# JuliaStats/Klara.jl

Measured on AMD Instinct MI355X. Metric: MCMC transitions/sec (whole node), 100-dim Gaussian, 65k chains, higher is better.
Workload: dtype f64

## Files before the change

### klara.jl_amd/csrc/detmath.h

```cpp
#ifndef KLARA_DETMATH_H
#define KLARA_DETMATH_H

#ifndef __HIPCC_RTC__
#include <stdint.h>
#endif

#if defined(__HIPCC__)
#define KD_FN __host__ __device__ __forceinline__
#else
#define KD_FN static inline __attribute__((always_inline))
#endif

KD_FN uint64_t kd_d2u(double x) { uint64_t u; __builtin_memcpy(&u, &x, 8); return u; }
KD_FN double   kd_u2d(uint64_t u) { double x; __builtin_memcpy(&x, &u, 8); return x; }
KD_FN double   kd_fma(double a, double b, double c) { return __builtin_fma(a, b, c); }

#define KD_PHILOX_M0 0xD2511F53u
#define KD_PHILOX_M1 0xCD9E8D57u
#define KD_PHILOX_W0 0x9E3779B9u
#define KD_PHILOX_W1 0xBB67AE85u

typedef struct { uint32_t x, y, z, w; } kd_u32x4;

#if defined(__HIP_DEVICE_COMPILE__)
// ... 374 lines not shown
    double d = kd_fma(-g, g, y);
    g = kd_fma(d, h, g);
    d = kd_fma(-g, g, y);
    return kd_fma(d, h, g);
#else
    return __builtin_sqrt(y);
#endif
}

KD_FN uint64_t kd_angle_bits20(uint32_t wb)
{
#if defined(__HIP_DEVICE_COMPILE__)
    return ((uint64_t)__builtin_amdgcn_alignbit(0x3ffu, wb, 12) << 32) | 0x80000000ull;
#else
    return ((uint64_t)(0x3ff00000u | (wb >> 12)) << 32) | 0x80000000ull;
#endif
}
#define KD_SCREM_ENTRIES 4096
#define KD_SCREM_BYTES (KD_SCREM_ENTRIES * 16)
KD_FN void kd_sincos_rem_entry(uint32_t m, double* sy_out, double* dc_out)
{
    kd_sincos_rem(kd_angle_bits20(m << 12), sy_out, dc_out);
}
#if defined(__HIPCC__)
typedef double kd_screm_t __attribute__((ext_vector_type(2)));
extern __shared__ __attribute__((aligned(16))) kd_screm_t kd_screm_lds[];
__device__ __forceinline__ void kd_sincos_rem_to_lds()
{
    for (int m = (int)threadIdx.x; m < KD_SCREM_ENTRIES; m += (int)blockDim.x) {
        double sy, dc;
        kd_sincos_rem_entry((uint32_t)m, &sy, &dc);
        kd_screm_lds[m] = kd_screm_t{ sy, dc };
    }
}
__device__ __forceinline__ void kd_sincos2pi_tab20(uint32_t wb, double* sn, double* cs)
{
    const uint32_t k = wb >> 12;
    const kd_screm_t r = kd_screm_lds[k & (KD_SCREM_ENTRIES - 1u)];
    kd_sincos_rotate(k >> 12, r.x, r.y, sn, cs);
}
#endif
#if defined(__HIPCC__)
template <bool TAB>
KD_FN void kd_normal_pair_w_t(uint32_t wa, uint32_t wb, double* z0, double* z1, double* u1_out, double* logu1_out)
#else
KD_FN void kd_normal_pair_w(uint32_t wa, uint32_t wb, double* z0, double* z1, double* u1_out, double* logu1_out)
#endif
{
    const double u1 = kd_u44(wa, wb);
    const double lg = kd_log_u01(u1);
    const double rad = kd_sqrt_radicand(-2.0 * lg);
    double sn, cs;
#if defined(__HIPCC__)
    if constexpr (TAB) kd_sincos2pi_tab20(wb, &sn, &cs);
    else
#endif
    kd_sincos2pi_bits(kd_angle_bits20(wb), &sn, &cs);
    *z0 = rad * cs;
    *z1 = rad * sn;
    *u1_out = u1;
    *logu1_out = lg;
}
#if defined(__HIPCC__)
KD_FN void kd_normal_pair_w(uint32_t wa, uint32_t wb, double* z0, double* z1, double* u1_out, double* logu1_out)
{
    kd_normal_pair_w_t<false>(wa, wb, z0, z1, u1_out, logu1_out);
}
#endif
#if defined(__HIPCC__)
typedef struct {
    kd_screm_t lg, rot, rem;
    double z; int k; double u1;
} kd_pair_reads;
__device__ __forceinline__ void kd_normal_pair_issue(uint32_t wa, uint32_t wb, kd_pair_reads* r)
{
    uint32_t i;
    r->u1 = kd_u44(wa, wb);
    kd_log_u01_reduce(r->u1, &i, &r->k, &r->z);
    const uint32_t k = wb >> 12;
    r->lg = *(const kd_screm_t*)&KD_LOGTAB(2 * i);
    r->rot = *(const kd_screm_t*)&KD_SCTAB(2 * (k >> 12));
    r->rem = kd_screm_lds[k & (KD_SCREM_ENTRIES - 1u)];
}
__device__ __forceinline__ void kd_normal_pair_finish(const kd_pair_reads* r, double* z0, double* z1, double* u1_out, double* logu1_out)
{
    const double lg = kd_log_u01_finish(r->z, r->k, r->lg.x, r->lg.y);
    const double rad = kd_sqrt_radicand(-2.0 * lg);
    double sn, cs;
    kd_sincos_rotate_entry(r->rot.x, r->rot.y, r->rem.x, r->rem.y, &sn, &cs);
    *z0 = rad * cs;
    *z1 = rad * sn;
    *u1_out = r->u1;
    *logu1_out = lg;
}
#endif

KD_FN uint32_t kd_pair_block(uint32_t p) { return (p & 7u) | ((p >> 4) << 3); }
KD_FN uint32_t kd_pair_half(uint32_t p) { return (p >> 3) & 1u; }
KD_FN void kd_normal_pair_at(uint64_t seed, uint64_t chain, uint64_t transition, uint32_t p, uint32_t nreal,
                             double* z0, double* z1, double* u1_out, double* logu1_out)
{
    const int real = p < nreal;
    const int half = real && kd_pair_half(p) != 0u;
    const kd_u32x4 b = kd_stream_block(seed, chain, transition, real ? kd_pair_block(p) : p);
    kd_normal_pair_w(half ? b.z : b.x, half ? b.w : b.y, z0, z1, u1_out, logu1_out);
}
KD_FN double kd_accept_uniform(kd_u32x4 b) { return kd_u44(b.x, b.y); }

KD_FN double kd_uniform_xy(kd_u32x4 b) { return kd_u52(b.x, b.y); }
KD_FN double kd_uniform_zw(kd_u32x4 b) { return kd_u52(b.z, b.w); }
KD_FN uint32_t kd_slice_attempt_slot(uint32_t base, uint32_t a) { return base | ((a + 1u) >> 1); }
KD_FN double kd_slice_attempt_uniform(uint64_t seed, uint64_t chain, uint64_t transition, uint32_t base, uint32_t a)
{
    const kd_u32x4 b = kd_stream_block(seed, chain, transition, kd_slice_attempt_slot(base, a));
    return (a & 1u) ? kd_uniform_xy(b) : kd_uniform_zw(b);
}

#endif
```

### klara.jl_amd/csrc/klara_diagt.h

```cpp
#pragma once
#include "klara_kernels.h"

#ifndef KLARA_DIAGT_Q
#define KLARA_DIAGT_Q 8
#endif
#define KLARA_DIAGT_CPW (64 / KLARA_DIAGT_Q)
#ifndef KLARA_DT_FENCE_EVERY
#define KLARA_DT_FENCE_EVERY 2
#endif
#ifndef KLARA_DT_SLICE_WF
#define KLARA_DT_SLICE_WF 4
#endif
#ifndef KLARA_DT_W1
#define KLARA_DT_W1 4
#endif
#ifndef KLARA_Q4_MALA_WF
#define KLARA_Q4_MALA_WF 3
#endif
#ifndef KLARA_Q4_SCTAB_WF
#define KLARA_Q4_SCTAB_WF 3
#endif
#ifndef KLARA_DT_WF
#define KLARA_DT_WF 2
#endif
#ifdef KLARA_DT_PERSISTENT
#define KLARA_DT_GROUP_LOOP for (long long grp = kl.group0 + wave0; grp < kl.group_end && grp * CPW < p.nchains; grp += nwaves)
#else
#define KLARA_DT_GROUP_LOOP const long long grp = kl.group0 + wave0; if (grp < kl.group_end && grp * CPW < p.nchains)
#endif
#define KLARA_DT_PAIR_FENCE(pi) do { if (KLARA_DT_FENCE_EVERY > 0 && ((pi) + 1) % KLARA_DT_FENCE_EVERY == 0) __builtin_amdgcn_sched_barrier(0); } while (0)

struct KAuto {
    const int* cell_in;
    int* cell_out;
    unsigned long long* acc_ctr;
    int* mirror;
    unsigned long long thr_work;
    int my_mode;
    int fanout;
    int launch_idx;
};
#define KLARA_AUTO_NONE KAuto{ nullptr, nullptr, nullptr, nullptr, 0ull, 0, 1, 0 }

__device__ __forceinline__ unsigned wave_sum_u32(unsigned v)
{
#pragma unroll
    for (int m = 1; m < 64; m <<= 1) v += (unsigned)__builtin_amdgcn_ds_bpermute((int)((((unsigned)threadIdx.x & 63u) ^ (unsigned)m) << 2), (int)v);
    return v;
}
__shared__ unsigned klara_auto_wg[2];
__device__ __forceinline__ void auto_begin()
{
    if (threadIdx.x < 2) klara_auto_wg[threadIdx.x] = 0u;
}
__device__ __forceinline__ void auto_finish(const KAuto& ka, unsigned wave_acc)
{
    if (ka.acc_ctr == nullptr) return;
    const unsigned tot = wave_sum_u32(wave_acc);
    if ((threadIdx.x & 63) == 0) {
        atomicAdd(&klara_auto_wg[0], tot);
        if (atomicAdd(&klara_auto_wg[1], 1u) != (blockDim.x >> 6) - 1) return;
        const unsigned long long wg_tot = atomicAdd(&klara_auto_wg[0], 0u);
        const unsigned long long old = atomicAdd(ka.acc_ctr, (1ull << 40) | wg_tot);
        if ((old >> 40) == (unsigned long long)gridDim.x - 1) {
            const unsigned long long total = (old & ((1ull << 40) - 1)) + wg_tot;
            *ka.acc_ctr = 0ull;
            const int mode = (total << 16) > ka.thr_work ? 1 : 0;
            if (ka.cell_out != nullptr) for (int k = 0; k < ka.fanout; ++k) ka.cell_out[2 * k] = mode;
            if (ka.mirror != nullptr) {
                for (int k = 0; k < ka.fanout; ++k) {
                    __hip_atomic_store(ka.mirror + 4 * k + 1, (int)(total > 0x7fffffffull ? 0x7fffffffull : total), __ATOMIC_RELAXED, __HIP_MEMORY_SCOPE_SYSTEM);
                    __hip_atomic_store(ka.mirror + 4 * k, mode, __ATOMIC_RELAXED, __HIP_MEMORY_SCOPE_SYSTEM);
                    __hip_atomic_store(ka.mirror + 4 * k + 2, ka.launch_idx, __ATOMIC_RELEASE, __HIP_MEMORY_SCOPE_SYSTEM);
                }
            }
        }
    }
}

template <int NP, int Q>
struct PairCtx {
    int lane, q, cw;
    unsigned off0;
    bool last_ok;
// ... 148 lines not shown
        }
#pragma unroll
        for (int k = 0; k < CH; ++k) {
            if (p0 + k < NP) {
                const int p = p0 + k;
                const unsigned o = fold ? pair_off<NP, Q>(c, p) : KLARA_BUF_OOB;
                const double s0 = __builtin_bit_cast(double, kd_uint2{ ts[k].x, ts[k].y }) + hf * x[2 * p];
                const double s1 = __builtin_bit_cast(double, kd_uint2{ ts[k].z, ts[k].w }) + hf * x[2 * p + 1];
                const double q0 = __builtin_bit_cast(double, kd_uint2{ tq[k].x, tq[k].y }) + hf * (x[2 * p] * x[2 * p]);
                const double q1 = __builtin_bit_cast(double, kd_uint2{ tq[k].z, tq[k].w }) + hf * (x[2 * p + 1] * x[2 * p + 1]);
                const kd_uint2 a = __builtin_bit_cast(kd_uint2, s0), b = __builtin_bit_cast(kd_uint2, s1);
                const kd_uint2 e = __builtin_bit_cast(kd_uint2, q0), f = __builtin_bit_cast(kd_uint2, q1);
                if (p < NP - 1) {
                    __builtin_amdgcn_raw_buffer_store_b128(kd_uint4{ a.x, a.y, b.x, b.y }, wsum, o, 0, 0);
                    __builtin_amdgcn_raw_buffer_store_b128(kd_uint4{ e.x, e.y, f.x, f.y }, wsq, o, 0, 0);
                } else {
                    const unsigned o1 = (fold && c.last_full) ? o + 8u : KLARA_BUF_OOB;
                    __builtin_amdgcn_raw_buffer_store_b64(a, wsum, o, 0, 0); __builtin_amdgcn_raw_buffer_store_b64(b, wsum, o1, 0, 0);
                    __builtin_amdgcn_raw_buffer_store_b64(e, wsq, o, 0, 0); __builtin_amdgcn_raw_buffer_store_b64(f, wsq, o1, 0, 0);
                }
            }
        }
    }
    held = fold ? 0 : held;
}

template <int NP, int Q>
__device__ __forceinline__ void load_pair_param(const PairCtx<NP, Q>& c, const gdouble* base, int D, double dflt, double (&v)[2 * NP])
{
#pragma unroll
    for (int p = 0; p < NP; ++p) {
        const int i = 2 * (p * Q + c.q);
        v[2 * p] = dflt; v[2 * p + 1] = dflt;
        if (base != nullptr && i < D) v[2 * p] = base[i];
        if (base != nullptr && i + 1 < D) v[2 * p + 1] = base[i + 1];
    }
}

template <int Q> struct PairShare {
    static constexpr int STEP = Q <= 8 ? 8 / Q : 0;
    static constexpr bool second(int p) { return STEP != 0 && ((p / (STEP ? STEP : 1)) & 1) != 0; }
};
template <int NP, int Q>
__device__ __forceinline__ void pair_words(const PairCtx<NP, Q>& c, unsigned long long seed, unsigned long long gchain,
                                           unsigned long long t, int p, uint32_t (&stash)[4], uint32_t& wa, uint32_t& wb)
{
    constexpr int STEP = PairShare<Q>::STEP, S1 = STEP ? STEP : 1;
    if (PairShare<Q>::second(p)) {
        wa = stash[2 * (p % S1)]; wb = stash[2 * (p % S1) + 1];
    } else {
        const uint32_t idx = (uint32_t)(p * Q + c.q);
        const bool pad = p == NP - 1 && !c.last_ok;
        const kd_u32x4 b = kd_stream_block(seed, gchain, t, pad ? idx : kd_pair_block(idx));
        if constexpr (STEP != 0) {
            wa = b.x; wb = b.y;
            stash[2 * (p % S1)] = b.z; stash[2 * (p % S1) + 1] = b.w;
        } else {
            const bool hb = !pad && kd_pair_half(idx) != 0u;
            wa = hb ? b.z : b.x; wb = hb ? b.w : b.y;
        }
    }
}
template <int NP, int Q, bool SCTAB = false>
__device__ __forceinline__ void pair_normals(const PairCtx<NP, Q>& c, unsigned long long seed, unsigned long long gchain,
                                             unsigned long long t, int p, uint32_t (&stash)[4], double& z0, double& z1, double& u1, double& lg1)
{
    uint32_t wa, wb;
    pair_words<NP, Q>(c, seed, gchain, t, p, stash, wa, wb);
    kd_normal_pair_w_t<SCTAB>(wa, wb, &z0, &z1, &u1, &lg1);
    KLARA_PIN(z0); KLARA_PIN(z1);
    if (p == NP - 1 && !c.last_ok) z0 = 0.0;
    if (p == NP - 1 && !c.last_full) z1 = 0.0;
}
template <int NP, int Q>
__device__ __forceinline__ void pair_issue(const PairCtx<NP, Q>& c, unsigned long long seed, unsigned long long gchain,
                                           unsigned long long t, int p, uint32_t (&stash)[4], kd_pair_reads& rd)
{
    uint32_t wa, wb;
    pair_words<NP, Q>(c, seed, gchain, t, p, stash, wa, wb);
    kd_normal_pair_issue(wa, wb, &rd);
    __builtin_amdgcn_sched_barrier(0);
}
template <int NP, int Q>
__device__ __forceinline__ void pair_finish(const PairCtx<NP, Q>& c, int p, const kd_pair_reads& rd, double& z0, double& z1, double& u1, double& lg1)
{
    kd_normal_pair_finish(&rd, &z0, &z1, &u1, &lg1);
    KLARA_PIN(z0); KLARA_PIN(z1);
    if (p == NP - 1 && !c.last_ok) z0 = 0.0;
    if (p == NP - 1 && !c.last_full) z1 = 0.0;
}

template <int V> struct kd_int { static constexpr int value = V; };
template <int FROM, int TO, class F>
__device__ __forceinline__ void kd_static_for(F&& f)
{
    if constexpr (FROM < TO) { f(kd_int<FROM>{}); kd_static_for<FROM + 1, TO>(f); }
}

template <bool UNITW>
__device__ __forceinline__ void diag_elem(double x, double w, double m2w, double m, double& term, double& grad)
{
    const double dd = UNITW ? x : x - m;
    term = UNITW ? dd * dd : w * (dd * dd);
    grad = UNITW ? -2.0 * dd : m2w * dd;
}

template <int SAMPLER, int NP, int Q, bool ONESTEP, bool TUNE, bool SCTAB = false>
__host__ __device__ constexpr int diagt_min_waves()
{
    return SCTAB && Q == 4 && NP > 8 ? KLARA_Q4_SCTAB_WF
         : NP <= 8 ? (ONESTEP && SAMPLER != KLARA_SAMPLER_HMC ? KLARA_DT_W1 : KLARA_DT_WF)
                   : (Q == 4 && NP <= 13 && !TUNE ? (SAMPLER == KLARA_SAMPLER_MALA ? KLARA_Q4_MALA_WF : 2) : 1);
}

#ifndef KLARA_SCTAB_MIN_STEPS
#define KLARA_SCTAB_MIN_STEPS 8
#endif
template <int SAMPLER, int NP, int Q, bool ONESTEP, bool UNITW, bool MON, bool TUNE>
__host__ __device__ constexpr bool diagt_sctab()
{
    return SAMPLER == KLARA_SAMPLER_MALA && ((Q == 4 && NP == 13) || (Q == 8 && NP == 7)) && !ONESTEP && UNITW && MON && !TUNE;
}
#ifndef KLARA_Q4_SCTAB_WG
#define KLARA_Q4_SCTAB_WG 256
#endif
template <int Q, bool SCTAB>
__host__ __device__ constexpr int diagt_wg_threads() { return SCTAB && Q == 4 ? KLARA_Q4_SCTAB_WG : 256; }
#ifndef KLARA_Q4_KEPT_MEANS
#define KLARA_Q4_KEPT_MEANS 0
#endif
#ifndef KLARA_Q8_KEPT_MEANS
#define KLARA_Q8_KEPT_MEANS 0
#endif
template <int SAMPLER, int NP, int Q, bool UNITW, bool TUNE, bool SCTAB>
__host__ __device__ constexpr int diagt_kept_means()
{
    return SCTAB && SAMPLER == KLARA_SAMPLER_MALA && UNITW && !TUNE ? (Q == 4 ? KLARA_Q4_KEPT_MEANS : Q == 8 ? KLARA_Q8_KEPT_MEANS : 0) : 0;
}

#ifdef KLARA_USER_PAIR_TARGET
#define KLARA_PAIR_CALL(a, b, P, g0, g1) klara_user_pair((a), (b), (P), D, (const double*)p.cdata, (long long)p.cndata, (g0), (g1))
#else
#define KLARA_PAIR_CALL(a, b, P, g0, g1) 0.0
#endif
template <int SAMPLER, int NP, int Q, bool ONESTEP, bool UNITW, bool MON, bool TUNE = false, bool DA = false, bool USERPAIR = false, bool SCTAB = false>
__global__ __launch_bounds__((diagt_wg_threads<Q, SCTAB>()), (SAMPLER == KLARA_SAMPLER_SLICE && NP <= 8 && !MON && !TUNE ? KLARA_DT_SLICE_WF : diagt_min_waves<SAMPLER, NP, Q, ONESTEP, TUNE, SCTAB>()))
void k_diagt(const KParams* __restrict__ pp, const KLaunch kl, const KAuto ka)
{
#ifndef KLARA_USER_PAIR_TARGET
    static_assert(!USERPAIR, "pair closures exist in run-time compiled translation units only");
#endif
    static_assert(!USERPAIR || (UNITW && Q >= 8), "pair closures: 8 or more lanes per chain");
    static_assert(!SCTAB || (!ONESTEP && !USERPAIR && SAMPLER != KLARA_SAMPLER_SLICE), "the remainder table: fused launches of the built-in MH / MALA / HMC kernels");
    if (ka.cell_in != nullptr && *ka.cell_in != ka.my_mode) return;
    static_assert(!(ONESTEP && (MON || TUNE)), "monitored / tuned jobs run the committing kernel");
    static_assert(!DA || (TUNE && SAMPLER == KLARA_SAMPLER_HMC), "dual averaging: tuned HMC");
    constexpr bool PLAIN = !TUNE;
    constexpr int E = 2 * NP, CPW = 64 / Q;
    constexpr bool NEEDG = SAMPLER == KLARA_SAMPLER_MALA || SAMPLER == KLARA_SAMPLER_HMC;
    constexpr bool SLICE = SAMPLER == KLARA_SAMPLER_SLICE;
    constexpr int KM = diagt_kept_means<SAMPLER, NP, Q, UNITW, TUNE, SCTAB>();
    static_assert(KM >= 0 && KM <= E, "kept drift means: a prefix of the lane's elements");
    static_assert(!(SLICE && ONESTEP), "the slice sampler moves every chain: it runs the committing kernel");
    constexpr bool MEMSUM = MON && !TUNE && Q == 4 && (SAMPLER == KLARA_SAMPLER_MH || SAMPLER == KLARA_SAMPLER_MALA);
    const KParams& p = *pp;
    __shared__ __attribute__((aligned(16))) double lds_w[UNITW ? 2 : 2 * NP * Q];
    __shared__ __attribute__((aligned(16))) double lds_mu[UNITW ? 2 : 2 * NP * Q];
    __shared__ __attribute__((aligned(16))) double lds_m2w[UNITW ? 2 : 2 * NP * Q];
    if (!UNITW) {
        for (int i = (int)threadIdx.x; i < 2 * NP * Q; i += (int)blockDim.x) {
            lds_w[i] = (p.gw != nullptr && i < p.D) ? p.gw[i] : 1.0;
            lds_mu[i] = (p.gmu != nullptr && i < p.D) ? p.gmu[i] : 0.0;
            lds_m2w[i] = -2.0 * lds_w[i];
        }
    }
    auto_begin();
    if constexpr (SCTAB) kd_sincos_rem_to_lds();
    kd_tables_to_lds();
    if (p.clock_probe != nullptr && blockIdx.x == (gridDim.x >> 1) && threadIdx.x == 0) {
        p.clock_probe[2] = __builtin_amdgcn_s_memtime(); p.clock_probe[3] = __builtin_amdgcn_s_memrealtime();
    }
    const int D = p.D;
    const PairCtx<NP, Q> cx = make_pctx<NP, Q>(D);
    const int nsteps = ONESTEP ? 1 : kl.nsteps;
    guchar* const accept_out = p.accept != nullptr ? p.accept + kl.t0 * (unsigned long long)p.nchains : nullptr;

    double sig[E];
    const auto wv = [&](int e) { return UNITW ? 1.0 : lds_w[2 * ((e >> 1) * Q + cx.q) + (e & 1)]; };
    const auto mv = [&](int e) { return UNITW ? 0.0 : lds_mu[2 * ((e >> 1) * Q + cx.q) + (e & 1)]; };
    const auto m2wv = [&](int e) { return UNITW ? -2.0 : lds_m2w[2 * ((e >> 1) * Q + cx.q) + (e & 1)]; };
    const auto wvl = [&](int e) { return UNITW ? 1.0 : *(volatile const double*)&lds_w[2 * ((e >> 1) * Q + cx.q) + (e & 1)]; };
    const auto mvl = [&](int e) { return UNITW ? 0.0 : *(volatile const double*)&lds_mu[2 * ((e >> 1) * Q + cx.q) + (e & 1)]; };
    const auto m2wvl = [&](int e) { return UNITW ? -2.0 : *(volatile const double*)&lds_m2w[2 * ((e >> 1) * Q + cx.q) + (e & 1)]; };
    if (SAMPLER == KLARA_SAMPLER_MH) load_pair_param<NP, Q>(cx, p.vecparam, D, 1.0, sig);
    const double gconst = USERPAIR ? 0.0 : p.gconst;

    const int acc_slot = (D + 1) >> 1;
    const bool acc_free = acc_slot < NP * Q && !PairShare<Q>::second(NP - 1);
    const int acc_lane = (cx.lane - cx.q) + (acc_slot & (Q - 1));

    const long long nwaves = (long long)gridDim.x * (blockDim.x >> 6);
    const long long wave0 = __builtin_amdgcn_readfirstlane((int)(blockIdx.x * (blockDim.x >> 6) + (threadIdx.x >> 6)));
    unsigned wave_acc = 0;
    KLARA_DT_GROUP_LOOP {
        const long long first_chain = grp * CPW;
        const long long left = p.nchains - first_chain;
        const int here = left < CPW ? (int)left : CPW;
        const bool chain_ok = cx.cw < here;
        const long long chain = first_chain + cx.cw;
        const unsigned long long gchain = (unsigned long long)(p.chain_offset + chain);
        const __amdgpu_buffer_rsrc_t wx = group_window(p.X, first_chain, here, D);
        const __amdgpu_buffer_rsrc_t wg = group_window(p.GR, first_chain, here, D);

        double x[E];
        load_pairs<NP, Q>(cx, wx, x);
        const auto late_ctx = [&]() -> PairCtx<NP, Q> {
            if constexpr (SCTAB && Q == 4) {
                int l = (int)__builtin_amdgcn_mbcnt_hi(~0u, __builtin_amdgcn_mbcnt_lo(~0u, 0u));
                KLARA_PIN(l);
                return make_pctx_at<NP, Q>(D, l & 63);
            } else return cx;
        };
        const auto user_pair = [&](int pi, double a, double b, double& nt, double& g0, double& g1) {
            double u0 = 0.0, u1 = 0.0, u = 0.0;
            const bool ok0 = pi < NP - 1 || cx.last_ok, ok1 = pi < NP - 1 || cx.last_full;
            if (ok0) u = KLARA_PAIR_CALL(a, b, pi * Q + cx.q, &u0, &u1);
            nt = ok0 ? -u : 0.0; g0 = ok0 ? u0 : 0.0; g1 = ok1 ? u1 : 0.0;
        };
        const auto grad_of = [&](const double (&v)[E], double (&out)[E]) {
            if constexpr (USERPAIR) {
#pragma unroll
                for (int pi = 0; pi < NP; ++pi) { double nt; user_pair(pi, v[2 * pi], v[2 * pi + 1], nt, out[2 * pi], out[2 * pi + 1]); }
            } else {
#pragma unroll
                for (int e = 0; e < E; ++e) { double term_; diag_elem<UNITW>(v[e], wv(e), m2wv(e), mv(e), term_, out[e]); }
            }
        };
        double lt = p.LT[chain_ok ? chain : 0];
        unsigned long long nacc = 0;
        bool stuck = false;
        const bool do_sum = MON && p.sum != nullptr;
        double sm[MEMSUM ? 2 : E], sq[MEMSUM ? 2 : E];
        bool sums_loaded = false;
        long long held = 0;
        __amdgpu_buffer_rsrc_t wsum = wx, wsq = wx;
        if (do_sum) {
#pragma unroll
            for (int e = 0; e < (MEMSUM ? 2 : E); ++e) { sm[e] = 0.0; sq[e] = 0.0; }
            wsum = group_window(p.sum, first_chain, here, D); wsq = group_window(p.sumsq, first_chain, here, D);
            held = p.held[chain_ok ? chain : 0];
        }
        int sphase = kl.save_phase0;
        long long scol = kl.save_col0;
        const bool per_chain_tune = KCNT && !KPOOLED;
        const long long c0 = chain_ok ? chain : 0;
        TuneRegs tn;
        if (per_chain_tune) tn = { p.tune_step[c0], p.tune_accepted[c0], p.tune_proposed[c0], p.tune_totproposed[c0], 0, 0.0, 0.0 };
        else if (KPOOLED) tn = { p.tune_step[0], p.tune_accepted[0], 0, 0, 0, 0.0, 0.0 };
        else tn = { DA ? p.tune_step[c0] : p.step0, 0, 0, 0, 0, 0.0, 0.0 };
        if (DA) { tn.epsbar = p.da_epsbar[c0]; tn.hbar = p.da_hbar[c0]; }
        const long long acc0 = tn.accepted;
        tn.phase = per_chain_tune ? (int)(tn.proposed % p.period) : 0;

        struct { unsigned long long seed; long long hist_cols, held_inc; int thinning, acc_free, save_lo, save_hi; double sqrt_step0, half_inv_step0; } lc = {};
        if constexpr (SCTAB) {
            lc.seed = p.seed; lc.hist_cols = p.hist_cols; lc.thinning = (int)p.thinning;
            lc.held_inc = __builtin_amdgcn_readfirstlane(do_sum ? 1 : 0); lc.sqrt_step0 = p.sqrt_step0;
            KLARA_PIN_S(lc.seed); KLARA_PIN_S(lc.hist_cols); KLARA_PIN_S(lc.thinning);
            KLARA_PIN_S(lc.held_inc); KLARA_PIN_S(lc.sqrt_step0);
            const kd_uint2 hih = __builtin_bit_cast(kd_uint2, 0.5 * p.inv_step0);
            lc.half_inv_step0 = __builtin_bit_cast(double, kd_uint2{ (uint32_t)__builtin_amdgcn_readfirstlane((int)hih.x), (uint32_t)__builtin_amdgcn_readfirstlane((int)hih.y) });
            KLARA_PIN_S(lc.half_inv_step0);
            lc.acc_free = __builtin_amdgcn_readfirstlane(acc_free ? 1 : 0);
            KLARA_PIN_S(lc.acc_free);
            const long long lo = (long long)p.burnin - (long long)kl.t0, hi = (long long)p.nsteps_total - (long long)kl.t0;
            lc.save_lo = (int)(lo < 0 ? 0 : lo > nsteps ? nsteps : lo); lc.save_hi = (int)(hi < 0 ? 0 : hi > nsteps ? nsteps : hi);
            KLARA_PIN_S(lc.save_lo); KLARA_PIN_S(lc.save_hi);
        }
#define KLARA_LC(f) (SCTAB ? lc.f : p.f)
        double dm[KM > 0 ? KM : 1];
        const double neg_h_kept = KM > 0 ? -tn.step : 0.0;
        if constexpr (KM > 0) {
#pragma unroll
            for (int e = 0; e < KM; ++e) dm[e] = x[e] + neg_h_kept * x[e];
        }
        for (int s = 0; s < nsteps; ++s) {
            const unsigned long long t = kl.t0 + (unsigned long long)s;
            if (KCNT) tune_count_proposal(p, tn);
            double xp[E];
            const auto put_xp = [&](int pi, double a, double b) { xp[2 * pi] = a; xp[2 * pi + 1] = b; };
            constexpr int NR = Q == 4 ? 2 : 1;
            double red[3 * NR] = {}, red1[1], red2[2];
            double u_last = 0.5, lg_last = 0.0;
            uint32_t nstash[4] = { 0u, 0u, 0u, 0u };
            bool acc;
            double ltp, a_da = 0.0;

            constexpr bool ZFIRST = (ONESTEP || Q != 4) && SAMPLER != KLARA_SAMPLER_HMC && !SLICE;
            double z[ZFIRST ? E : 2];
            kd_pair_reads rd[2];
            if (ZFIRST) {
                if constexpr (SCTAB) pair_issue<NP, Q>(cx, KLARA_LC(seed), gchain, t, 0, nstash, rd[0]);
#pragma unroll
                for (int pi = 0; pi < NP; ++pi) {
                    if constexpr (SCTAB) {
                        if (pi + 1 < NP) pair_issue<NP, Q>(cx, KLARA_LC(seed), gchain, t, pi + 1, nstash, rd[(pi + 1) & 1]);
                        pair_finish<NP, Q>(cx, pi, rd[pi & 1], z[2 * pi], z[2 * pi + 1], u_last, lg_last);
                        __builtin_amdgcn_sched_barrier(0);
                    } else {
                        pair_normals<NP, Q, SCTAB>(cx, KLARA_LC(seed), gchain, t, pi, nstash, z[2 * pi], z[2 * pi + 1], u_last, lg_last);
                        KLARA_DT_PAIR_FENCE(pi);
                    }
                }
            }
            if constexpr (SLICE) {
                if (do_sum && __any(held > 0))
                    diagt_fold<NP, Q>(cx, wsum, wsq, held > 0, sums_loaded, held, x, sm, sq);
            }
            if (SLICE) {
                acc = true;
                const __amdgpu_buffer_rsrc_t wwid = __builtin_amdgcn_make_buffer_rsrc((void*)p.vecparam, 0, D * 8, 0x00020000);
#pragma unroll
                for (int e = 0; e < E; ++e) {
                    const int i = 2 * ((e >> 1) * Q + cx.q) + (e & 1);
                    const bool live = chain_ok && i < D;
                    const uint32_t base = (uint32_t)(live ? i : 0) << KLARA_SLICE_ATT_BITS;
                    const kd_u32x4 b0 = kd_stream_block(KLARA_LC(seed), gchain, t, base);
                    const double lgu = kd_log_u01(kd_uniform_xy(b0));
                    const double ru = kd_uniform_zw(b0);
                    const double wi_t = UNITW ? 1.0 : wv(e), mi_t = UNITW ? 0.0 : mv(e);
                    const double xi = x[e], wd = __builtin_bit_cast(double, __builtin_amdgcn_raw_buffer_load_b64(wwid, (unsigned)(live ? i : 0) * 8u, 0, 0));
                    double tcur, gd_;
                    if constexpr (USERPAIR) { double g1_; user_pair(e >> 1, x[e & ~1], x[e | 1], tcur, gd_, g1_); }
                    else diag_elem<UNITW>(xi, wi_t, -2.0 * wi_t, mi_t, tcur, gd_);
                    double Li = xi - ru * wd;
                    double Ri = xi + (1.0 - ru) * wd;
                    const auto term_of = [&](double cand) -> double {
                        double tc, gd;
                        if constexpr (USERPAIR) { double g1; user_pair(e >> 1, (e & 1) ? x[e & ~1] : cand, (e & 1) ? cand : x[e | 1], tc, gd, g1); }
                        else diag_elem<UNITW>(cand, wi_t, -2.0 * wi_t, mi_t, tc, gd);
                        return tc;
                    };
                    if (p.stepout) {
                        double dl = tcur - term_of(Li);
                        int guard = 0;
                        while (true) {
                            bool go = live && !stuck && (dl > lgu);
                            if (go && ++guard > KLARA_SLICE_MAX_ATT) { stuck = true; go = false; }
                            if (!__any(go)) break;
                            const double Ln = Li - wd;
                            const double dn = tcur - term_of(go ? Ln : Li);
                            if (go) { Li = Ln; dl = dn; }
                        }
                        double dr = tcur - term_of(Ri);
                        guard = 0;
                        while (true) {
                            bool go = live && !stuck && (dr > lgu);
                            if (go && ++guard > KLARA_SLICE_MAX_ATT) { stuck = true; go = false; }
                            if (!__any(go)) break;
                            const double Rn = Ri + wd;
                            const double dn = tcur - term_of(go ? Rn : Ri);
                            if (go) { Ri = Rn; dr = dn; }
                        }
                    }
                    double xprime = xi;
                    bool done = !live || stuck;
                    kd_u32x4 ab = b0;
// ... 5 lines not shown
                        const double cand = u * (Ri - Li) + Li;
                        const double tc = term_of(done ? xprime : cand);
                        if (!done) {
                            xprime = cand;
                            if (tcur - tc > lgu) done = true;
                            else if (cand > xi) Ri = cand;
                            else if (cand < xi) Li = cand;
                            else { stuck = true; done = true; }
                        }
                    }
                    if (live && !stuck) x[e] = xprime;
                }
                red1[0] = 0.0;
                if constexpr (USERPAIR) {
#pragma unroll
                    for (int pi = 0; pi < NP; ++pi) { double nt, g0_, g1_; user_pair(pi, x[2 * pi], x[2 * pi + 1], nt, g0_, g1_); red1[0] = red1[0] + nt; }
                } else {
#pragma unroll
                for (int e = 0; e < E; ++e) { double te, gd; diag_elem<UNITW>(x[e], wv(e), m2wv(e), mv(e), te, gd); red1[0] = red1[0] + te; }
                }
                group_allreduce<1>(red1, Q, cx.lane);
                lt = gconst - red1[0];
                ltp = lt;
#pragma unroll
                for (int e = 0; e < E; ++e) xp[e] = x[e];
            } else if (SAMPLER == KLARA_SAMPLER_MH) {
                const auto mh_elem = [&](int e, double ze, int r) -> double {
                    const double xe = x[e] + sig[e] * ze;
                    double term, gd;
                    diag_elem<UNITW>(xe, wv(e), m2wv(e), mv(e), term, gd);
                    red[r] = red[r] + term;
                    return xe;
                };
#pragma unroll
                for (int pi = 0; pi < NP; ++pi) {
                    double z0 = ZFIRST ? z[(2 * pi) % (ZFIRST ? E : 2)] : 0.0, z1 = ZFIRST ? z[(2 * pi + 1) % (ZFIRST ? E : 2)] : 0.0;
                    if (!ZFIRST) pair_normals<NP, Q, SCTAB>(cx, KLARA_LC(seed), gchain, t, pi, nstash, z0, z1, u_last, lg_last);
                    const int r = (NR == 2 && (pi & 1)) ? 3 : 0;
                    if constexpr (USERPAIR) {
                        const double a = x[2 * pi] + sig[2 * pi] * z0, b = x[2 * pi + 1] + sig[2 * pi + 1] * z1;
                        double nt, g0, g1;
                        user_pair(pi, a, b, nt, g0, g1);
                        red[r] = red[r] + nt;
                        put_xp(pi, a, b);
                    } else {
                        const double a = mh_elem(2 * pi, z0, r), b = mh_elem(2 * pi + 1, z1, r);
                        put_xp(pi, a, b);
                    }
                    if (!ZFIRST) KLARA_DT_PAIR_FENCE(pi);
                }
                if (NR == 2) {
                    red2[0] = red[0]; red2[1] = red[3];
                    group_allreduce<2>(red2, Q, cx.lane);
                    red1[0] = red2[0] + red2[1];
                } else {
                    red1[0] = red[0];
                    group_allreduce<1>(red1, Q, cx.lane);
                }
                ltp = gconst - red1[0];
                const double ratio = ltp - lt;
                acc = ratio > 0.0;
                if (acc_free) acc = acc || ratio > lane_bcast(lg_last, acc_lane);
                else if (!acc && ratio > KD_LOG_UMIN_GUARD)
                    acc = ratio > kd_log_u01(kd_accept_uniform(kd_stream_block(KLARA_LC(seed), gchain, t, (uint32_t)acc_slot)));
            } else if (SAMPLER == KLARA_SAMPLER_MALA) {
                const double h_ = tn.step, halfh = 0.5 * h_, sq = KCNT ? __builtin_sqrt(h_) : KLARA_LC(sqrt_step0);
                const double half_inv_h = SCTAB ? lc.half_inv_step0 : 0.5 * (KCNT ? 1.0 / h_ : p.inv_step0);
                const double neg_h = -h_;
                constexpr bool FROM_TERM = UNITW && PLAIN;
                const auto mala_elem = [&](int e, double ze, int r, bool first) -> double {
                    double term, ge = 0.0, gpe;
                    if constexpr (!UNITW) diag_elem<UNITW>(x[e], wv(e), m2wv(e), mv(e), term, ge);
                    const double m_ = UNITW ? (e < KM ? dm[e < KM ? e : 0] : x[e] + neg_h * x[e]) : x[e] + halfh * ge;
                    const double xe = m_ + sq * ze;
                    diag_elem<UNITW>(xe, wv(e), m2wv(e), mv(e), term, gpe);
                    red[r] = first ? term : red[r] + term;
                    const double q1 = m_ - xe;
                    red[r + 1] = first ? (q1 * q1) * half_inv_h : red[r + 1] + (q1 * q1) * half_inv_h;
                    const double mup = UNITW ? xe + neg_h * xe : xe + halfh * gpe;
                    const double q2 = mup - x[e];
                    red[r + 2] = first ? (q2 * q2) * half_inv_h : red[r + 2] + (q2 * q2) * half_inv_h;
                    return xe;
                };
#pragma unroll
                for (int pi = 0; pi < NP; ++pi) {
                    double z0 = ZFIRST ? z[(2 * pi) % (ZFIRST ? E : 2)] : 0.0, z1 = ZFIRST ? z[(2 * pi + 1) % (ZFIRST ? E : 2)] : 0.0;
                    if constexpr (!ZFIRST && SCTAB) {
                        if (pi == 0) pair_issue<NP, Q>(cx, KLARA_LC(seed), gchain, t, 0, nstash, rd[0]);
                        pair_finish<NP, Q>(cx, pi, rd[pi & 1], z0, z1, u_last, lg_last);
                        if (pi + 1 < NP) pair_issue<NP, Q>(cx, KLARA_LC(seed), gchain, t, pi + 1, nstash, rd[(pi + 1) & 1]);
                    } else if (!ZFIRST) pair_normals<NP, Q, SCTAB>(cx, KLARA_LC(seed), gchain, t, pi, nstash, z0, z1, u_last, lg_last);
                    const int r = (NR == 2 && (pi & 1)) ? 3 : 0;
                    if constexpr (USERPAIR) {
                        double nt, ge0, ge1, gp0, gp1;
                        user_pair(pi, x[2 * pi], x[2 * pi + 1], nt, ge0, ge1);
                        const double m0 = x[2 * pi] + halfh * ge0, m1 = x[2 * pi + 1] + halfh * ge1;
                        const double a = m0 + sq * z0, b = m1 + sq * z1;
                        user_pair(pi, a, b, nt, gp0, gp1);
                        red[r] = red[r] + nt;
                        const double q10 = m0 - a, q11 = m1 - b;
                        red[r + 1] = red[r + 1] + (q10 * q10) * half_inv_h;
                        red[r + 1] = red[r + 1] + (q11 * q11) * half_inv_h;
                        const double q20 = (a + halfh * gp0) - x[2 * pi], q21 = (b + halfh * gp1) - x[2 * pi + 1];
                        red[r + 2] = red[r + 2] + (q20 * q20) * half_inv_h;
                        red[r + 2] = red[r + 2] + (q21 * q21) * half_inv_h;
                        put_xp(pi, a, b);
                    } else {
                        const double a = mala_elem(2 * pi, z0, r, FROM_TERM && pi < NR), b = mala_elem(2 * pi + 1, z1, r, false);
                        put_xp(pi, a, b);
                    }
                    if constexpr (!ZFIRST && SCTAB) __builtin_amdgcn_sched_barrier(0);
                    else if (!ZFIRST) KLARA_DT_PAIR_FENCE(pi);
                }
                group_allreduce<3 * NR>(red, Q, cx.lane);
                if (NR == 2) { red[0] = red[0] + red[3]; red[1] = red[1] + red[4]; red[2] = red[2] + red[5]; }
                ltp = gconst - red[0];
                double ratio = ltp - lt;
                ratio += red[1];
                ratio -= red[2];
                acc = ratio > 0.0;
                if (SCTAB ? lc.acc_free != 0 : acc_free) acc = acc || ratio > lane_bcast(lg_last, acc_lane);
                else {
                    double guard = KD_LOG_UMIN_GUARD;
                    if constexpr (SCTAB) KLARA_PIN_S(guard);
                    if (!acc && ratio > guard)
                        acc = ratio > kd_log_u01(kd_accept_uniform(kd_stream_block(KLARA_LC(seed), gchain, t, (uint32_t)acc_slot)));
                }
            } else {
                const double eps = tn.step, halfe = 0.5 * eps;
                double mom[E], gp[E];
                double k0[NR] = {};
#pragma unroll
                for (int pi = 0; pi < NP; ++pi) {
                    pair_normals<NP, Q, SCTAB>(cx, KLARA_LC(seed), gchain, t, pi, nstash, mom[2 * pi], mom[2 * pi + 1], u_last, lg_last);
                    const int r = (NR == 2 && (pi & 1)) ? 1 : 0;
                    k0[r] = k0[r] + mom[2 * pi] * mom[2 * pi];
                    k0[r] = k0[r] + mom[2 * pi + 1] * mom[2 * pi + 1];
                }
                group_allreduce<NR>(k0, Q, cx.lane);
                if (NR == 2) k0[0] = k0[0] + k0[1];
                const double H0 = lt - 0.5 * k0[0];
#pragma unroll
                for (int e = 0; e < E; ++e) xp[e] = x[e];
                constexpr bool KFOLD = UNITW && !USERPAIR;
                if constexpr (!KFOLD) grad_of(x, gp);
                const int nl = DA ? (chain_ok ? da_nleaps(p, eps) : 1) : p.nleaps;
#pragma unroll
                for (int e = 0; e < E; ++e) {
                    if constexpr (KFOLD) mom[e] = kd_fma(-eps, x[e], mom[e]);
                    else mom[e] = kd_fma(halfe, gp[e], mom[e]);
                }
                const int nlmax = DA ? wave_max_int(nl) : nl;
                for (int l = 0; l < nlmax; ++l) {
                    const bool go = !DA || l < nl;
                    const double kf = l + 1 < nl ? eps : halfe;
                    const double nkf2 = -2.0 * kf;
                    if constexpr (USERPAIR) {
#pragma unroll
                        for (int pi = 0; pi < NP; ++pi) {
                            const double xa = kd_fma(eps, mom[2 * pi], xp[2 * pi]), xb = kd_fma(eps, mom[2 * pi + 1], xp[2 * pi + 1]);
                            xp[2 * pi] = go ? xa : xp[2 * pi]; xp[2 * pi + 1] = go ? xb : xp[2 * pi + 1];
                            double nt, ga, gb;
                            user_pair(pi, xp[2 * pi], xp[2 * pi + 1], nt, ga, gb);
                            gp[2 * pi] = go ? ga : gp[2 * pi]; gp[2 * pi + 1] = go ? gb : gp[2 * pi + 1];
                            const double na = kd_fma(kf, gp[2 * pi], mom[2 * pi]), nb = kd_fma(kf, gp[2 * pi + 1], mom[2 * pi + 1]);
                            mom[2 * pi] = go ? na : mom[2 * pi]; mom[2 * pi + 1] = go ? nb : mom[2 * pi + 1];
                        }
                    } else {
#pragma unroll
                        for (int e = 0; e < E; ++e) {
                            const double x1 = kd_fma(eps, mom[e], xp[e]);
                            xp[e] = go ? x1 : xp[e];
                            if constexpr (KFOLD) {
                                const double m2 = kd_fma(nkf2, xp[e], mom[e]);
                                mom[e] = go ? m2 : mom[e];
                            } else {
                                double term, g1;
                                diag_elem<UNITW>(xp[e], 1.0, m2wvl(e), mvl(e), term, g1);
                                gp[e] = go ? g1 : gp[e];
                                const double m2 = kd_fma(kf, gp[e], mom[e]);
                                mom[e] = go ? m2 : mom[e];
                            }
                        }
                    }
                }
                if constexpr (USERPAIR) {
#pragma unroll
                    for (int pi = 0; pi < NP; ++pi) {
                        double nt, ga, gb;
                        user_pair(pi, xp[2 * pi], xp[2 * pi + 1], nt, ga, gb);
                        red[0] = red[0] + nt;
                        red[1] = red[1] + mom[2 * pi] * mom[2 * pi];
                        red[1] = red[1] + mom[2 * pi + 1] * mom[2 * pi + 1];
                    }
                } else {
#pragma unroll
                for (int e = 0; e < E; ++e) {
                    double term, gd;
                    diag_elem<UNITW>(xp[e], wv(e), m2wv(e), mv(e), term, gd);
                    const int r = (NR == 2 && ((e >> 1) & 1)) ? 3 : 0;
                    red[r] = red[r] + term;
                    red[r + 1] = red[r + 1] + mom[e] * mom[e];
                }
                }
                if (NR == 2) {
                    double red4[4] = { red[0], red[1], red[3], red[4] };
                    group_allreduce<4>(red4, Q, cx.lane);
                    red2[0] = red4[0] + red4[2]; red2[1] = red4[1] + red4[3];
                } else {
                    red2[0] = red[0]; red2[1] = red[1];
                    group_allreduce<2>(red2, Q, cx.lane);
                }
                ltp = gconst - red2[0];
                const double H1 = ltp - 0.5 * red2[1];
                const double ratio = H1 - H0;
                const double ex = kd_exp(ratio);
                const double a = 1.0 < ex ? 1.0 : ex;
                a_da = a;
                const double u = acc_free ? lane_bcast(u_last, acc_lane)
                                          : kd_accept_uniform(kd_stream_block(KLARA_LC(seed), gchain, t, (uint32_t)acc_slot));
                acc = u < a;
            }

            if constexpr (SCTAB) {
                if (accept_out != nullptr) {
                    const PairCtx<NP, Q> cxa = late_ctx();
                    if (cxa.cw < here && cxa.q == 0) accept_out[(long long)s * p.nchains + (first_chain + cxa.cw)] = acc ? 1 : 0;
                }
            } else if (accept_out != nullptr && chain_ok && cx.q == 0) accept_out[(long long)s * p.nchains + chain] = acc ? 1 : 0;
            if (KCNT && acc && !SLICE) tn.accepted += 1;
            if (DA) da_update(p, tn, (long long)t + 1, a_da);
            if (per_chain_tune && !DA) tuning_block(p, tn);
            else if (DA && per_chain_tune && tn.phase == 0 && (long long)t + 1 <= p.da_nadapt) {
                tn.totproposed += tn.proposed; tn.accepted = 0; tn.proposed = 0;
            }
            if constexpr (ONESTEP) {
                wave_acc += (acc && chain_ok && cx.q == 0) ? 1u : 0u;
                if (acc) {
                    store_pairs<NP, Q>(cx, wx, xp);
                    if (NEEDG) { double gq[E]; grad_of(xp, gq); store_pairs<NP, Q>(cx, wg, gq); }
                    if (chain_ok && cx.q == 0) { p.LT[chain] = ltp; p.naccept[chain] += 1ull; }
                }
            } else {
                nacc += acc ? 1ull : 0ull;
                if (!SLICE && do_sum && __any(chain_ok && acc && held > 0)) {
                    const bool fold = chain_ok && acc && held > 0;
#ifdef KLARA_DT_FOLD_RMW
                    if constexpr (MEMSUM) diagt_fold_rmw<NP, Q>(cx, wsum, wsq, fold, held, x);
#else
                    if constexpr (MEMSUM) diagt_fold_atomic<NP, Q>(cx, p.sum + first_chain * D, p.sumsq + first_chain * D, fold, held, x);
#endif
                    else diagt_fold<NP, Q>(cx, wsum, wsq, fold, sums_loaded, held, x, sm, sq);
                }
                if (acc) {
#pragma unroll
                    for (int e = 0; e < E; ++e) x[e] = xp[e];
                    if constexpr (KM > 0) {
#pragma unroll
                        for (int e = 0; e < KM; ++e) dm[e] = xp[e] + neg_h_kept * xp[e];
                    }
                    lt = ltp;
                }
            }
            const long long i1 = (long long)t + 1;
            if (MON && (SCTAB ? s >= lc.save_lo && s < lc.save_hi : i1 > p.burnin && i1 <= p.nsteps_total)) {
                if (sphase == 0) {
                    if constexpr (SCTAB) held += lc.held_inc;
                    else if (do_sum) held += 1;
                    if (scol < KLARA_LC(hist_cols)) {
                        const long long col0 = scol * p.nchains + first_chain;
                        const PairCtx<NP, Q> cxh = late_ctx();
                        if (p.hist != nullptr) store_pairs<NP, Q>(cxh, group_window(p.hist, col0, here, D), x);
                        if (NEEDG && p.hist_g != nullptr) { double gq[E]; grad_of(x, gq); store_pairs<NP, Q>(cxh, group_window(p.hist_g, col0, here, D), gq); }
                        if constexpr (SCTAB) {
                            if (p.hist_lt != nullptr && cxh.cw < here && cxh.q == 0) p.hist_lt[scol * p.nchains + (first_chain + cxh.cw)] = lt;
                        } else if (p.hist_lt != nullptr && chain_ok && cx.q == 0) p.hist_lt[scol * p.nchains + chain] = lt;
                    }
                    ++scol;
                }
                sphase = (sphase + 1 == (SCTAB ? lc.thinning : (int)p.thinning)) ? 0 : sphase + 1;
            }
        }
        const PairCtx<NP, Q> cxe = late_ctx();
        const bool chain_ok_e = SCTAB ? cxe.cw < here : chain_ok;
        const long long chain_e = SCTAB ? first_chain + cxe.cw : chain;
        if (do_sum) {
            if constexpr (!MEMSUM) {
                if (__any(sums_loaded)) {
                    store_pairs_if<NP, Q>(cxe, wsum, sums_loaded, sm);
                    store_pairs_if<NP, Q>(cxe, wsq, sums_loaded, sq);
                }
            }
            if (chain_ok_e && cxe.q == 0) p.held[chain_e] = held;
        }
        if (SLICE && stuck && chain_ok) klara_raise(p.error_flag, KLARA_ERR_SLICE_STUCK);
        if (!ONESTEP) wave_acc += (chain_ok_e && cxe.q == 0) ? (unsigned)nacc : 0u;
        if (!ONESTEP && nacc != 0) {
            store_pairs<NP, Q>(cxe, wx, x);
            if (NEEDG) { double gq[E]; grad_of(x, gq); store_pairs<NP, Q>(cxe, wg, gq); }
            if (chain_ok_e && cxe.q == 0) { p.LT[chain_e] = lt; p.naccept[chain_e] += nacc; }
        }
        if (TUNE && chain_ok && cx.q == 0) {
            if (DA) { p.tune_step[chain] = tn.step; p.da_epsbar[chain] = tn.epsbar; p.da_hbar[chain] = tn.hbar; }
            if (per_chain_tune) {
                p.tune_step[chain] = tn.step; p.tune_accepted[chain] = tn.accepted;
                p.tune_proposed[chain] = tn.proposed; p.tune_totproposed[chain] = tn.totproposed;
            } else if (KPOOLED && KCNT) {
                atomicAdd((unsigned long long*)p.pooled_accepted, (unsigned long long)(tn.accepted - acc0));
            }
        }
    }
    if (p.clock_probe != nullptr && blockIdx.x == (gridDim.x >> 1) && threadIdx.x == 0) {
        p.clock_probe[0] = __builtin_amdgcn_s_memtime(); p.clock_probe[1] = __builtin_amdgcn_s_memrealtime();
    }
    auto_finish(ka, wave_acc);
#undef KLARA_LC
}

template <int NP, int Q, bool USERPAIR = false>
__global__ __launch_bounds__(256) void k_diagt_init(const KParams p, int needgrad)
{
#ifndef KLARA_USER_PAIR_TARGET
    static_assert(!USERPAIR, "pair closures exist in run-time compiled translation units only");
#endif
    constexpr int E = 2 * NP, CPW = 64 / Q;
    const int D = p.D;
    const PairCtx<NP, Q> cx = make_pctx<NP, Q>(D);
    const long long grp = __builtin_amdgcn_readfirstlane((int)(blockIdx.x * (blockDim.x >> 6) + (threadIdx.x >> 6)));
    const long long first_chain = grp * CPW;
    const long long left = p.nchains - first_chain;
    const int here = left < CPW ? (left > 0 ? (int)left : 0) : CPW;
    const bool chain_ok = cx.cw < here;
    const long long chain = first_chain + cx.cw;
    double w[E], mu[E], x[E], g[E], red[1] = { 0.0 };
    load_pair_param<NP, Q>(cx, p.gw, D, 1.0, w);
    load_pair_param<NP, Q>(cx, p.gmu, D, 0.0, mu);
    load_pairs<NP, Q>(cx, group_window(p.X, first_chain, here, D), x);
    bool bad = false;
    if constexpr (USERPAIR) {
#pragma unroll
        for (int pi = 0; pi < NP; ++pi) {
            double u0 = 0.0, u1 = 0.0, u = 0.0;
// ... 23 lines not shown
```

Baseline: 6.213 billion.

## Add closed-form MALA rejection screen to skip full proposal evaluation

For the Q=4, NP=13 MALA fused path, the normals are first drawn while accumulating x·x, x·z and z·z. A closed-form estimate of the log acceptance ratio, with a rigorous error bound, then decides whether every chain in the wave is certainly rejected. When the screen is certain, the per-element drift and target evaluation plus the reduction are skipped, and a run limit forces a full evaluation periodically. The normal-pair reads are also split into log and angle halves to interleave table loads, and the accept counter is narrowed to 32 bits. The cost is extra register pressure and a two-value reduction on every step.

New measurement: 6.973 billion (median of 6 runs). 12.2% higher.

```diff
diff --git a/klara.jl_amd/csrc/detmath.h b/klara.jl_amd/csrc/detmath.h
--- a/klara.jl_amd/csrc/detmath.h
+++ b/klara.jl_amd/csrc/detmath.h
@@ -480,6 +480,19 @@
     r->rot = *(const kd_screm_t*)&KD_SCTAB(2 * (k >> 12));
     r->rem = kd_screm_lds[k & (KD_SCREM_ENTRIES - 1u)];
 }
+__device__ __forceinline__ void kd_normal_pair_issue_log(uint32_t wa, uint32_t wb, kd_pair_reads* r)
+{
+    uint32_t i;
+    r->u1 = kd_u44(wa, wb);
+    kd_log_u01_reduce(r->u1, &i, &r->k, &r->z);
+    r->lg = *(const kd_screm_t*)&KD_LOGTAB(2 * i);
+}
+__device__ __forceinline__ void kd_normal_pair_issue_angle(uint32_t wb, kd_pair_reads* r)
+{
+    const uint32_t k = wb >> 12;
+    r->rot = *(const kd_screm_t*)&KD_SCTAB(2 * (k >> 12));
+    r->rem = kd_screm_lds[k & (KD_SCREM_ENTRIES - 1u)];
+}
 __device__ __forceinline__ void kd_normal_pair_finish(const kd_pair_reads* r, double* z0, double* z1, double* u1_out, double* logu1_out)
 {
     const double lg = kd_log_u01_finish(r->z, r->k, r->lg.x, r->lg.y);
diff --git a/klara.jl_amd/csrc/klara_diagt.h b/klara.jl_amd/csrc/klara_diagt.h
--- a/klara.jl_amd/csrc/klara_diagt.h
+++ b/klara.jl_amd/csrc/klara_diagt.h
@@ -1,5 +1,6 @@
 #pragma once
 #include "klara_kernels.h"
+#include "klara_mala_screen.h"
 
 #ifndef KLARA_DIAGT_Q
 #define KLARA_DIAGT_Q 8
@@ -314,6 +315,20 @@
     __builtin_amdgcn_sched_barrier(0);
 }
 template <int NP, int Q>
+__device__ __forceinline__ void pair_issue_log(const PairCtx<NP, Q>& c, unsigned long long seed, unsigned long long gchain,
+                                               unsigned long long t, int p, uint32_t (&stash)[4], kd_pair_reads& rd, uint32_t& wb)
+{
+    uint32_t wa;
+    pair_words<NP, Q>(c, seed, gchain, t, p, stash, wa, wb);
+    kd_normal_pair_issue_log(wa, wb, &rd);
+    __builtin_amdgcn_sched_barrier(0);
+}
+__device__ __forceinline__ void pair_issue_angle(uint32_t wb, kd_pair_reads& rd)
+{
+    kd_normal_pair_issue_angle(wb, &rd);
+    __builtin_amdgcn_sched_barrier(0);
+}
+template <int NP, int Q>
 __device__ __forceinline__ void pair_finish(const PairCtx<NP, Q>& c, int p, const kd_pair_reads& rd, double& z0, double& z1, double& u1, double& lg1)
 {
     kd_normal_pair_finish(&rd, &z0, &z1, &u1, &lg1);
@@ -352,6 +367,19 @@
 __host__ __device__ constexpr bool diagt_sctab()
 {
     return SAMPLER == KLARA_SAMPLER_MALA && ((Q == 4 && NP == 13) || (Q == 8 && NP == 7)) && !ONESTEP && UNITW && MON && !TUNE;
+}
+#ifndef KLARA_MALA_SCREEN
+#define KLARA_MALA_SCREEN 1
+#endif
+#ifndef KLARA_MALA_SCREEN_RUN
+#define KLARA_MALA_SCREEN_RUN 2
+#endif
+template <bool C, class A, class B> struct kd_type_if { typedef A type; };
+template <class A, class B> struct kd_type_if<false, A, B> { typedef B type; };
+template <int SAMPLER, int NP, int Q, bool UNITW, bool TUNE, bool USERPAIR, bool SCTAB>
+__host__ __device__ constexpr bool diagt_mala_screen()
+{
+    return KLARA_MALA_SCREEN != 0 && SCTAB && SAMPLER == KLARA_SAMPLER_MALA && Q == 4 && NP == 13 && UNITW && !TUNE && !USERPAIR;
 }
 #ifndef KLARA_Q4_SCTAB_WG
 #define KLARA_Q4_SCTAB_WG 256
@@ -393,6 +421,7 @@
     constexpr bool SLICE = SAMPLER == KLARA_SAMPLER_SLICE;
     constexpr int KM = diagt_kept_means<SAMPLER, NP, Q, UNITW, TUNE, SCTAB>();
     static_assert(KM >= 0 && KM <= E, "kept drift means: a prefix of the lane's elements");
+    constexpr bool SCREEN = diagt_mala_screen<SAMPLER, NP, Q, UNITW, TUNE, USERPAIR, SCTAB>();
     static_assert(!(SLICE && ONESTEP), "the slice sampler moves every chain: it runs the committing kernel");
     constexpr bool MEMSUM = MON && !TUNE && Q == 4 && (SAMPLER == KLARA_SAMPLER_MH || SAMPLER == KLARA_SAMPLER_MALA);
     const KParams& p = *pp;
@@ -404,6 +433,14 @@
             lds_w[i] = (p.gw != nullptr && i < p.D) ? p.gw[i] : 1.0;
             lds_mu[i] = (p.gmu != nullptr && i < p.D) ? p.gmu[i] : 0.0;
             lds_m2w[i] = -2.0 * lds_w[i];
+        }
+    }
+    __shared__ __attribute__((aligned(16))) double lds_screen[6];
+    if constexpr (SCREEN) {
+        if (threadIdx.x == 0) {
+            const kd_mala_screen_k k = kd_mala_screen_consts(p.step0, p.sqrt_step0, 0.5 * p.inv_step0);
+            lds_screen[0] = k.K0; lds_screen[1] = k.K1; lds_screen[4] = k.K2; lds_screen[5] = 0.0;
+            lds_screen[2] = k.on ? k.T0 : __builtin_nan(""); lds_screen[3] = k.on ? k.T2 : __builtin_nan("");
         }
     }
     auto_begin();
@@ -469,7 +506,7 @@
             }
         };
         double lt = p.LT[chain_ok ? chain : 0];
-        unsigned long long nacc = 0;
+        typename kd_type_if<SCREEN, unsigned, unsigned long long>::type nacc = 0;
         bool stuck = false;
         const bool do_sum = MON && p.sum != nullptr;
         double sm[MEMSUM ? 2 : E], sq[MEMSUM ? 2 : E];
@@ -515,6 +552,12 @@
         if constexpr (KM > 0) {
 #pragma unroll
             for (int e = 0; e < KM; ++e) dm[e] = x[e] + neg_h_kept * x[e];
+        }
+        double sxx = 0.0;
+        int srun = 0;
+        if constexpr (SCREEN) {
+#pragma unroll
+            for (int e = 0; e < E; ++e) sxx = kd_fma(x[e], x[e], sxx);
         }
         for (int s = 0; s < nsteps; ++s) {
             const unsigned long long t = kl.t0 + (unsigned long long)s;
@@ -686,10 +729,48 @@
                     red[r + 2] = first ? (q2 * q2) * half_inv_h : red[r + 2] + (q2 * q2) * half_inv_h;
                     return xe;
                 };
+                bool screened = false;
+                if constexpr (SCREEN) {
+                    double sxz = 0.0, szz = 0.0;
+                    kd_screm_t sk01, skt;
+                    double sk2;
+                    pair_issue<NP, Q>(cx, KLARA_LC(seed), gchain, t, 0, nstash, rd[0]);
+#pragma unroll
+                    for (int pi = 0; pi < NP; ++pi) {
+                        double z0, z1;
+                        uint32_t wb_next = 0u;
+                        if (pi == NP - 1) {
+                            typedef volatile const __attribute__((address_space(3))) kd_screm_t* lds_entry;
+                            sk01 = *(lds_entry)&lds_screen[0]; skt = *(lds_entry)&lds_screen[2];
+                            sk2 = *(volatile const __attribute__((address_space(3))) double*)&lds_screen[4];
+                            __builtin_amdgcn_sched_barrier(0);
+                        }
+                        if (pi + 1 < NP) pair_issue_log<NP, Q>(cx, KLARA_LC(seed), gchain, t, pi + 1, nstash, rd[(pi + 1) & 1], wb_next);
+                        pair_finish<NP, Q>(cx, pi, rd[pi & 1], z0, z1, u_last, lg_last);
+                        if (pi + 1 < NP) pair_issue_angle(wb_next, rd[(pi + 1) & 1]);
+                        sxz = kd_fma(x[2 * pi], z0, sxz); sxz = kd_fma(x[2 * pi + 1], z1, sxz);
+                        szz = kd_fma(z0, z0, szz); szz = kd_fma(z1, z1, szz);
+                        put_xp(pi, z0, z1);
+                        __builtin_amdgcn_sched_barrier(0);
+                    }
+                    double sc[2] = { kd_mala_screen_e(sk01.x, sk01.y, sk2, sxx, sxz, szz), kd_mala_screen_t(skt.x, skt.y, sxx, szz) };
+                    group_allreduce<2>(sc, Q, cx.lane);
+                    double lg_s;
+                    if (lc.acc_free != 0) lg_s = lane_bcast(lg_last, acc_lane);
+                    else { lg_s = KD_LOG_UMIN_GUARD; KLARA_PIN_S(lg_s); }
+                    const bool certain = !chain_ok || kd_mala_screen_decide(sc[0], sc[1], lt, gconst, lg_s, nullptr, nullptr) != 0;
+                    screened = __all(certain) != 0;
+                    if (KLARA_MALA_SCREEN_RUN > 0 && srun >= KLARA_MALA_SCREEN_RUN) screened = false;
+                    srun = screened ? srun + 1 : 0;
+                    KLARA_PIN(srun);
+                    acc = false; ltp = lt;
+                }
+                if (!screened) {
 #pragma unroll
                 for (int pi = 0; pi < NP; ++pi) {
                     double z0 = ZFIRST ? z[(2 * pi) % (ZFIRST ? E : 2)] : 0.0, z1 = ZFIRST ? z[(2 * pi + 1) % (ZFIRST ? E : 2)] : 0.0;
-                    if constexpr (!ZFIRST && SCTAB) {
+                    if constexpr (SCREEN) { z0 = xp[2 * pi]; z1 = xp[2 * pi + 1]; }
+                    else if constexpr (!ZFIRST && SCTAB) {
                         if (pi == 0) pair_issue<NP, Q>(cx, KLARA_LC(seed), gchain, t, 0, nstash, rd[0]);
                         pair_finish<NP, Q>(cx, pi, rd[pi & 1], z0, z1, u_last, lg_last);
                         if (pi + 1 < NP) pair_issue<NP, Q>(cx, KLARA_LC(seed), gchain, t, pi + 1, nstash, rd[(pi + 1) & 1]);
@@ -713,7 +794,8 @@
                         const double a = mala_elem(2 * pi, z0, r, FROM_TERM && pi < NR), b = mala_elem(2 * pi + 1, z1, r, false);
                         put_xp(pi, a, b);
                     }
-                    if constexpr (!ZFIRST && SCTAB) __builtin_amdgcn_sched_barrier(0);
+                    if constexpr (SCREEN) { }
+                    else if constexpr (!ZFIRST && SCTAB) __builtin_amdgcn_sched_barrier(0);
                     else if (!ZFIRST) KLARA_DT_PAIR_FENCE(pi);
                 }
                 group_allreduce<3 * NR>(red, Q, cx.lane);
@@ -729,6 +811,7 @@
                     if constexpr (SCTAB) KLARA_PIN_S(guard);
                     if (!acc && ratio > guard)
                         acc = ratio > kd_log_u01(kd_accept_uniform(kd_stream_block(KLARA_LC(seed), gchain, t, (uint32_t)acc_slot)));
+                }
                 }
             } else {
                 const double eps = tn.step, halfe = 0.5 * eps;
@@ -846,7 +929,7 @@
                     if (chain_ok && cx.q == 0) { p.LT[chain] = ltp; p.naccept[chain] += 1ull; }
                 }
             } else {
-                nacc += acc ? 1ull : 0ull;
+                nacc += acc ? 1u : 0u;
                 if (!SLICE && do_sum && __any(chain_ok && acc && held > 0)) {
                     const bool fold = chain_ok && acc && held > 0;
 #ifdef KLARA_DT_FOLD_RMW
@@ -862,6 +945,11 @@
                     if constexpr (KM > 0) {
 #pragma unroll
                         for (int e = 0; e < KM; ++e) dm[e] = xp[e] + neg_h_kept * xp[e];
+                    }
+                    if constexpr (SCREEN) {
+                        sxx = 0.0;
+#pragma unroll
+                        for (int e = 0; e < E; ++e) sxx = kd_fma(xp[e], xp[e], sxx);
                     }
                     lt = ltp;
                 }
diff --git a/klara.jl_amd/csrc/klara_mala_screen.h b/klara.jl_amd/csrc/klara_mala_screen.h
--- /dev/null
+++ b/klara.jl_amd/csrc/klara_mala_screen.h
@@ -0,0 +1,64 @@
+#ifndef KLARA_MALA_SCREEN_H
+#define KLARA_MALA_SCREEN_H
+
+#include "detmath.h"
+
+#define KD_MALA_SCREEN_H_MIN 0.015625
+#define KD_MALA_SCREEN_H_MAX 2.0
+#define KD_MALA_SCREEN_MARGIN 9.313225746154785e-10
+#define KD_MALA_SCREEN_T_MAX 1.0715086071862673e+301
+#define KD_MALA_SCREEN_ELEM_FACTOR 96.0
+
+typedef struct {
+    double K0, K1, K2;
+    double T0, T2;
+    int on;
+} kd_mala_screen_k;
+
+KD_FN double kd_mala_screen_abs(double v) { return __builtin_fabs(v); }
+
+KD_FN kd_mala_screen_k kd_mala_screen_consts(double h, double s, double c)
+{
+    kd_mala_screen_k k;
+    const double a = 1.0 - h, a2 = a * a, b = a2 - 1.0, aa = kd_mala_screen_abs(a), ab = kd_mala_screen_abs(b);
+    const double cb = c * b, one_cb = 1.0 + cb, s2 = s * s;
+    k.K0 = -(a2 + cb * b);
+    k.K1 = -2.0 * (a * s) * one_cb;
+    k.K2 = -s2 * one_cb;
+    const double cross = c * ab * aa * s;
+    k.T0 = a2 + aa * s + c * (b * b) + cross;
+    k.T2 = s2 + aa * s + c * s2 + cross + c * (a2 * s2);
+    const double mu = h + aa;
+    const double exz = s * (16.0 * mu + 8.0 * aa + c * mu * (8.0 + 6.0 * mu * aa));
+    const double E0 = 11.0 * (mu * mu) + 4.0 * ab + 0.5 * exz;
+    const double E2 = 5.0 * s2 + 4.0 + 2.0 * a2 + 3.0 * mu * aa + 0.5 * exz;
+    const double tiny = 8.881784197001252e-16;
+    int on = h >= KD_MALA_SCREEN_H_MIN && h <= KD_MALA_SCREEN_H_MAX;
+    on = on && kd_mala_screen_abs(s2 - h) <= tiny * h && kd_mala_screen_abs(c * h - 0.5) <= tiny;
+    on = on && k.T0 >= 0.25 && k.T2 >= 0.25;
+    on = on && E0 <= KD_MALA_SCREEN_ELEM_FACTOR * k.T0 && E2 <= KD_MALA_SCREEN_ELEM_FACTOR * k.T2;
+    k.on = on;
+    return k;
+}
+
+KD_FN double kd_mala_screen_e(double K0, double K1, double K2, double sxx, double sxz, double szz) { return kd_fma(K0, sxx, kd_fma(K1, sxz, K2 * szz)); }
+KD_FN double kd_mala_screen_t(double T0, double T2, double sxx, double szz) { return kd_fma(T0, sxx, T2 * szz); }
+
+KD_FN int kd_mala_screen_decide(double e, double ts, double lt, double gconst, double lg, double* est_out, double* t_out)
+{
+    const double est = (gconst - lt) + e;
+    const double T = ((kd_mala_screen_abs(gconst) + kd_mala_screen_abs(lt)) + kd_mala_screen_abs(lg)) + ts;
+    if (est_out) *est_out = est;
+    if (t_out) *t_out = T;
+    return (T <= KD_MALA_SCREEN_T_MAX) && (est + KD_MALA_SCREEN_MARGIN * T <= lg);
+}
+
+KD_FN int kd_mala_screen_certain(const kd_mala_screen_k* k, double sxx, double sxz, double szz, double lt, double gconst, double lg,
+                                 double* est_out, double* t_out)
+{
+    const int r = kd_mala_screen_decide(kd_mala_screen_e(k->K0, k->K1, k->K2, sxx, sxz, szz), kd_mala_screen_t(k->T0, k->T2, sxx, szz),
+                                        lt, gconst, lg, est_out, t_out);
+    return k->on && r;
+}
+
+#endif
```
